# kamenbliznashki/chexpert

Measured on AMD Instinct MI355X. Metric: images/sec fwd+bwd DenseNet121 320x320 bf16 (per-GPU rate in config.images_per_sec_per_gpu), higher is better.
Workload: dtype bf16; 1 GPU; densenet121 bf16 1xMI355X 320x320 bs=256 per GPU, U-Ones labels (BASELINE configs[1]); 14 classes; random-init weights, synthetic uint8 X-rays; per_gpu_batch=256, global_batch=256, parallelism=dp1, rccl_ranks=1, capture_failed=0, launch=hipGraph replay

## Files before the change

chexpert_amd/csrc/conv3x3_ring.hip:

```cpp
#include <cstdlib>
#include <type_traits>
#include "common.h"

namespace {

constexpr int XP = 272;
constexpr int NT = 512;
constexpr int W_ROWS = 9 * 32;
constexpr int W_BYTES = W_ROWS * XP;
constexpr int RING_PX_MAX = (160 * 1024 - W_BYTES - 1024 - 256) / XP;

struct RingGeo {
  int B, H, W, P, R, Q;
  int Wt, ntx;
  int spi;
  int steps_per_wg;
  unsigned mP;
  unsigned mSpi;
  int ntx_shift;
};

__device__ __forceinline__ int wrapq(int v, int q) { return v >= q ? v - q : v; }
__device__ __forceinline__ int div_spi(const RingGeo& g, int v) { return g.spi == 1 ? v : (int)__umulhi((unsigned)v, g.mSpi); }

template <int CTRL>
__device__ __forceinline__ float dpp_add(float v) {
  return v + __int_as_float(__builtin_amdgcn_update_dpp(0, __float_as_int(v), CTRL, 0xF, 0xF, true));
}
__device__ __forceinline__ float half_sum(float v) {
  v = dpp_add<0xB1>(v);
  v = dpp_add<0x4E>(v);
  v = dpp_add<0x141>(v);
  v = dpp_add<0x140>(v);
  return v + __shfl_xor(v, 16);
}

#ifdef CX_RING_STAMPS
__device__ unsigned long long ring_stamps[1024 * 8];
__device__ unsigned long long ring_fwd_stamps[1024 * 8];
__device__ __forceinline__ unsigned long long rstamp() {
  unsigned long long t;
  __builtin_amdgcn_sched_barrier(0);
  asm volatile("s_memtime %0\n\ts_waitcnt lgkmcnt(0)" : "=s"(t)::"memory");
  __builtin_amdgcn_sched_barrier(0);
  return t;
}
#define RSTAMP(i) { const unsigned long long t_ = rstamp(); st_acc[i] += t_ - st_prev; st_prev = t_; }
#else
#define RSTAMP(i)
#endif
template <int NCH, int DEPTH>
__global__ __launch_bounds__(NT, 1) void conv3x3_ring_fwd_kernel(const bf16* __restrict__ x, int ldx, const float* __restrict__ sc,
                                                                const float* __restrict__ sh, const bf16* __restrict__ wpk,
                                                                bf16* __restrict__ y, int ldy, float* stat_sum, float* stat_sq,
                                                                int stat_replicas, int stat_rstride, int stat_det, const RingGeo g) {
  extern __shared__ __attribute__((aligned(16))) char smem[];
  float* coef = reinterpret_cast<float*>(smem);
  char* wl = smem + 1024 + 256;
  char* ring = wl + W_BYTES;
  const int tid = threadIdx.x, lane = tid & 63, wave = tid >> 6;
  const int lrow = lane & 31, lh = lane >> 5;
  const int P = g.P, R = g.R, Q = g.Q, W = g.W, H = g.H, Wt = g.Wt, ntx = g.ntx;

  for (int i = tid; i < W_ROWS * 16; i += NT) {
    const int row = i >> 4, c = i & 15;
    *reinterpret_cast<uint4*>(wl + row * XP + c * 16) = *reinterpret_cast<const uint4*>(wpk + (size_t)row * 128 + c * 8);
  }
  for (int i = tid; i < (Q + 2) * (XP / 16); i += NT) reinterpret_cast<uint4*>(ring)[i] = make_uint4(0, 0, 0, 0);
  __syncthreads();

  const int total_steps = g.B * g.spi;
  const int u0 = blockIdx.x * g.steps_per_wg;
  const int u1 = min(total_steps, u0 + g.steps_per_wg);
  const int chunks_per_row = P * 16;

  uint4 pre[DEPTH][NCH];
  bool pv[DEPTH][NCH];
  int base_row = 0;
  int crow[NCH], cpx[NCH];
  const int cc8 = tid & 15;
#pragma unroll
  for (int i = 0; i < NCH; ++i) {
    const int cid = tid + NT * i;
    crow[i] = cid / chunks_per_row;
    cpx[i] = (cid - crow[i] * chunks_per_row) >> 4;
  }
  float csc[8], csh[8];
#pragma unroll
  for (int j = 0; j < 8; ++j) { csc[j] = sc[cc8 * 8 + j]; csh[j] = sh[cc8 * 8 + j]; }
#pragma unroll
  for (int j = 0; j < 8; ++j) asm volatile("" ::"v"(csc[j]), "v"(csh[j]));
  uint32_t voff[NCH];
#pragma unroll
  for (int i = 0; i < NCH; ++i) voff[i] = ((uint32_t)(crow[i] * W + cpx[i]) * (uint32_t)ldx + (uint32_t)cc8 * 8u) * 2u;
  const char* __restrict__ xb = reinterpret_cast<const char*>(x);
  auto issue_rows = [&](uint4 (&pre)[NCH], bool (&pv)[NCH], int bv, int y0, int n) __attribute__((always_inline)) {
    const int b = bv >> g.ntx_shift, x0 = (bv - (b << g.ntx_shift)) * Wt - 1;
    const uint32_t sbase = (uint32_t)((b * H + y0) * W + x0) * (uint32_t)ldx * 2u;
    const uint32_t r_lo = (uint32_t)max(-y0, 0), r_n = (uint32_t)max(min(n, H - y0), 0) - r_lo;
    const uint32_t c_lo = (uint32_t)max(-x0, 0), c_n = (uint32_t)max(W - x0, 0) - c_lo;
#pragma unroll
    for (int i = 0; i < NCH; ++i) {
      pv[i] = ((uint32_t)crow[i] - r_lo) < r_n && ((uint32_t)cpx[i] - c_lo) < c_n;
      pre[i] = *reinterpret_cast<const uint4*>(xb + (size_t)(pv[i] ? sbase + voff[i] : 0u));
    }
  };
  auto write_rows = [&](uint4 (&pre)[NCH], bool (&pv)[NCH], int y0, int n) __attribute__((always_inline)) {
    int slot_y0 = (y0 - base_row) % (R + 2);
    if (slot_y0 < 0) slot_y0 += R + 2;
#pragma unroll
    for (int i = 0; i < NCH; ++i) {
      if (crow[i] < n) {
        int slot = slot_y0 + crow[i];
        if (slot >= R + 2) slot -= R + 2;
        U128 o;
        o.u = cx_affine_relu8(pre[i], csc, csh);
        { const unsigned keep = pv[i] ? 0xffffffffu : 0u; o.u.x &= keep; o.u.y &= keep; o.u.z &= keep; o.u.w &= keep; }
        const int pos = slot * P + cpx[i];
        *reinterpret_cast<uint4*>(ring + pos * XP + cc8 * 16) = o.u;
        if (pos < 2) *reinterpret_cast<uint4*>(ring + (Q + pos) * XP + cc8 * 16) = o.u;
      }
    }
  };
  int ulim = u1;
  auto issue_step = [&](uint4 (&pre)[NCH], bool (&pv)[NCH], int v) __attribute__((always_inline)) {
    const int bv = div_spi(g, v), sv = v - bv * g.spi;
    const bool ok = v < ulim && sv != 0;
    issue_rows(pre, pv, ok ? bv : 0, ok ? sv * R + 1 : 0, ok ? R : 0);
  };

  float s1[2][8], s2[2][8];
#pragma unroll
  for (int cc = 0; cc < 2; ++cc)
#pragma unroll
    for (int j = 0; j < 8; ++j) s1[cc][j] = s2[cc][j] = 0.f;
  const int nsub = (R * P + 31) / 32;
  const char* wbase = wl + lrow * XP + lh * 16;
#ifdef CX_RING_STAMPS
  unsigned long long st_acc[7] = {0, 0, 0, 0, 0, 0, 0}, st_prev = rstamp(), st_steps = 0;
#endif

  auto step = [&](int u, auto KI) __attribute__((always_inline)) {
    constexpr int k = decltype(KI)::value;
    uint4 (&cur)[NCH] = pre[k];
    bool (&cv)[NCH] = pv[k];
    const int bv = div_spi(g, u), yc = (u - bv * g.spi) * R;
    const int b = bv >> g.ntx_shift, x0 = (bv - (b << g.ntx_shift)) * Wt;
    RSTAMP(0)
    write_rows(cur, cv, yc + 1, R);
    RSTAMP(1)
    __syncthreads();
    RSTAMP(2)
    issue_step(cur, cv, u + DEPTH);
    RSTAMP(3)
    int slot0 = (yc - 1 - base_row) % (R + 2);
    if (slot0 < 0) slot0 += R + 2;
    const int ws = slot0 * P;

    for (int s = wave; s < nsub; s += NT / 64) {
      f32x16 acc;
#pragma unroll
      for (int r = 0; r < 16; ++r) acc[r] = 0.f;
      const int m = s * 32 + lrow;
      const int pix = min(m, R * P - 1);
      const char* ap0 = ring + wrapq(wrapq(ws + pix, Q), Q) * XP + lh * 16;
      const char* ap1 = ring + wrapq(wrapq(ws + pix + P, Q), Q) * XP + lh * 16;
      const char* ap2 = ring + wrapq(wrapq(ws + pix + 2 * P, Q), Q) * XP + lh * 16;
      constexpr int G = 3, NG = 72 / G;
      bf16x8 fa[3][G], fb[3][G];
      auto load_grp = [&](int gi, bf16x8 (&A)[G], bf16x8 (&B)[G]) __attribute__((always_inline)) {
#pragma unroll
        for (int j = 0; j < G; ++j) {
          const int f = gi * G + j, t = f >> 3, ks = f & 7;
          const int dy = t / 3, dx = t - dy * 3;
          A[j] = *reinterpret_cast<const bf16x8*>(wbase + t * 32 * XP + ks * 32);
          B[j] = *reinterpret_cast<const bf16x8*>((dy == 0 ? ap0 : dy == 1 ? ap1 : ap2) + dx * XP + ks * 32);
        }
      };
      load_grp(0, fa[0], fb[0]);
      load_grp(1, fa[1], fb[1]);
#pragma unroll
      for (int gi = 0; gi < NG; ++gi) {
        if (gi + 2 < NG) load_grp(gi + 2, fa[(gi + 2) % 3], fb[(gi + 2) % 3]);
        __builtin_amdgcn_sched_barrier(0);
#pragma unroll
        for (int j = 0; j < G; ++j)
          acc = __builtin_amdgcn_mfma_f32_32x32x16_bf16(fa[gi % 3][j], fb[gi % 3][j], acc, 0, 0, 0);
        __builtin_amdgcn_sched_barrier(0);
      }
#ifdef CX_RING_STAMPS
      asm volatile("" ::"v"(acc[0]));
#endif
      RSTAMP(4)
      const int oy = (int)__umulhi((unsigned)m, g.mP), ox = m - oy * P;
      const int yy = yc + oy;
      const bool valid = m < R * P && ox < Wt && x0 + ox < W && yy < H;
      bf16* yrow = y + ((size_t)(b * H + (valid ? yy : 0)) * W + (valid ? x0 + ox : 0)) * ldy;
#pragma unroll
      for (int cc = 0; cc < 2; ++cc) {
        U128 o;
        float t[8];
#pragma unroll
        for (int r4 = 0; r4 < 4; ++r4) {
          const auto sw = __builtin_amdgcn_permlane32_swap(__float_as_uint(acc[8 * cc + r4]), __float_as_uint(acc[8 * cc + 4 + r4]),
                                                           false, false);
          t[r4] = __uint_as_float(sw[0]);
          t[4 + r4] = __uint_as_float(sw[1]);
        }
        o.u = cx_pack8_stats(t, valid, true, s1[cc], s2[cc]);
        if (valid) *reinterpret_cast<uint4*>(yrow + 8 * (2 * cc + lh)) = o.u;
      }
      RSTAMP(5)
    }
    __syncthreads();
    RSTAMP(6)
#ifdef CX_RING_STAMPS
    ++st_steps;
#endif
  };

  const int rot = u1 - u0 > 1 ? (int)((blockIdx.x * 37u) % (unsigned)(u1 - u0)) : 0;
#pragma unroll 1
  for (int pass = 0; pass < 2; ++pass) {
  ulim = pass == 0 ? u1 : u0 + rot;
  for (int ui = pass == 0 ? u0 + rot : u0; ui < ulim;) {
    const int b = div_spi(g, ui), yc = (ui - b * g.spi) * R;
    const int ue = min(ulim, (b + 1) * g.spi);
    base_row = yc - 1;
    auto sync_rows = [&](int y0) __attribute__((always_inline)) {
      issue_rows(pre[0], pv[0], b, y0, 1);
      write_rows(pre[0], pv[0], y0, 1);
    };
    sync_rows(yc - 1);
    sync_rows(yc);
    issue_rows(pre[0], pv[0], b, yc + 1, R);
#pragma unroll
    for (int d = 1; d < DEPTH; ++d) issue_step(pre[d], pv[d], ui + d);
    for (int u = ui; u < ue; u += DEPTH) {
      step(u, std::integral_constant<int, 0>());
      if (DEPTH > 1) { if (u + 1 >= ue) break; step(u + 1, std::integral_constant<int, 1 % DEPTH>()); }
      if (DEPTH > 2) { if (u + 2 >= ue) break; step(u + 2, std::integral_constant<int, 2 % DEPTH>()); }
    }
    ui = ue;
  }
  }

#ifdef CX_RING_STAMPS
  if (tid == 0 && blockIdx.x < 1024) {
    for (int i = 0; i < 7; ++i) ring_fwd_stamps[blockIdx.x * 8 + i] = st_acc[i];
    ring_fwd_stamps[blockIdx.x * 8 + 7] = st_steps;
  }
#endif
  if (stat_sum) {
    float* scratch = reinterpret_cast<float*>(wl);
    wg_stat_begin<NT / 64>(scratch, 32, tid, NT);
    float t1 = 0.f, t2 = 0.f;
#pragma unroll
    for (int cc = 0; cc < 2; ++cc)
#pragma unroll
      for (int j = 0; j < 8; ++j) {
        const float a = half_sum(s1[cc][j]);
        const float c = half_sum(s2[cc][j]);
        if (lrow == 8 * cc + j) { t1 = a; t2 = c; }
      }
    if (lrow < 16) {
      const int n = 8 * (2 * (lrow >> 3) + lh) + (lrow & 7);
      wg_stat_put(scratch, 32, wave, n, t1, t2);
    }
    wg_stat_end<NT / 64>(scratch, 32, tid, NT, stat_sum, stat_sq, stat_det, (int)blockIdx.x, stat_replicas, stat_rstride, 0, 32);
  }
}

template <int NCH, int DEPTH>
int launch_ring(const CxConv& p, hipStream_t st, const RingGeo& g) {
  const size_t smem = 1024 + 256 + W_BYTES + (size_t)(g.Q + 2) * XP;
  static bool attr = false;
  if (!attr) {
    (void)hipFuncSetAttribute(reinterpret_cast<const void*>(&conv3x3_ring_fwd_kernel<NCH, DEPTH>), hipFuncAttributeMaxDynamicSharedMemorySize,
                              160 * 1024);
    attr = true;
  }
  const int total = g.B * g.spi;
  const int grid = (total + g.steps_per_wg - 1) / g.steps_per_wg;
  if (const int e = stat_rows_check(p, grid)) return e;
  CX_KTAG("conv3x3_ring_fwd_kernel<%d, %d>", NCH, DEPTH);
  hipLaunchKernelGGL((conv3x3_ring_fwd_kernel<NCH, DEPTH>), dim3(grid), dim3(NT), smem, st, (const bf16*)p.x, p.ldx, p.pa, p.pb,
                     (const bf16*)p.w, (bf16*)p.y, p.ldy, p.stat_sum, p.stat_sq, p.stat_replicas, p.stat_rstride, p.stat_det, g);
  return launch_status();
}


constexpr int GP = 80;
constexpr int DW_ROWS = 9 * 128;
constexpr int DW_BYTES = DW_ROWS * GP;
constexpr int EC_BYTES = 5 * 128 * 4 + 3 * 32 * 4;
constexpr int MAX_ITEMS = 2;

template <int NCH>
__global__ __launch_bounds__(NT, 1) void conv3x3_ring_dgrad_kernel(
    const bf16* __restrict__ gsl, int ldg, const bf16* __restrict__ g2, int ldg2, const float* __restrict__ ga,
    const float* __restrict__ gb, const float* __restrict__ gc, const bf16* __restrict__ wpk, const bf16* __restrict__ ex, int ldex,
    const float* __restrict__ e_sc, const float* __restrict__ e_sh, const float* __restrict__ e_mu, const float* __restrict__ e_r,
    const float* __restrict__ e_scale, bf16* __restrict__ y, int ldy, float* S1, float* S2, int stat_replicas, int stat_rstride,
    int stat_det, bf16* __restrict__ po, int ldpo, const RingGeo g) {
  extern __shared__ __attribute__((aligned(16))) char smem[];
  float* ecoef = reinterpret_cast<float*>(smem);
  char* wl = smem + EC_BYTES;
  char* ring = wl + DW_BYTES;
  const int tid = threadIdx.x, lane = tid & 63, wave = tid >> 6;
  const int lrow = lane & 31, lh = lane >> 5;
  const int h2 = wave & 1;
  const int P = g.P, R = g.R, Q = g.Q, W = g.W, H = g.H;

  for (int i = tid; i < DW_ROWS * 4; i += NT) {
    const int row = i >> 2, c = i & 3;
    *reinterpret_cast<uint4*>(wl + row * GP + c * 16) = *reinterpret_cast<const uint4*>(wpk + (size_t)row * 32 + c * 8);
  }
  for (int i = tid; i < (Q + 2) * (GP / 16); i += NT) reinterpret_cast<uint4*>(ring)[i] = make_uint4(0, 0, 0, 0);
  if (tid < 128) {
    ecoef[tid] = e_sc[tid]; ecoef[128 + tid] = e_sh[tid]; ecoef[256 + tid] = e_mu[tid]; ecoef[384 + tid] = e_r[tid];
    ecoef[512 + tid] = e_scale[tid];
  }
  if (tid < 32) { ecoef[640 + tid] = ga[tid]; ecoef[672 + tid] = gb[tid]; ecoef[704 + tid] = gc[tid]; }
  __syncthreads();

  const int total_steps = g.B * g.spi;
  const int u0 = blockIdx.x * g.steps_per_wg;
  const int u1 = min(total_steps, u0 + g.steps_per_wg);
  const int cpr = W * 4;

  uint4 pg[NCH], pg2[NCH];
  bool gv[NCH];
  int base_row = 0;
  int crow[NCH], cpx[NCH];
  const int cc4 = tid & 3;
#pragma unroll
  for (int i = 0; i < NCH; ++i) {
    const int cid = tid + NT * i;
    crow[i] = cid / cpr;
    cpx[i] = (cid - crow[i] * cpr) >> 2;
  }
  const float* kco = ecoef + 640 + cc4 * 8;

  uint32_t vog[NCH], vog2[NCH];
#pragma unroll
  for (int i = 0; i < NCH; ++i) {
    vog[i] = ((uint32_t)(crow[i] * W + cpx[i]) * (uint32_t)ldg + (uint32_t)cc4 * 8u) * 2u;
    vog2[i] = ((uint32_t)(crow[i] * W + cpx[i]) * (uint32_t)ldg2 + (uint32_t)cc4 * 8u) * 2u;
  }
  const char* __restrict__ gslb = reinterpret_cast<const char*>(gsl);
  const char* __restrict__ g2b = reinterpret_cast<const char*>(g2);
  auto issue_rows = [&](int b, int y0, int n) __attribute__((always_inline)) {
    const uint32_t row0 = (uint32_t)((b * H + y0) * W);
    const uint32_t sg = row0 * (uint32_t)ldg * 2u, sg2 = row0 * (uint32_t)ldg2 * 2u;
    const uint32_t r_lo = (uint32_t)max(-y0, 0), r_n = (uint32_t)max(min(n, H - y0), 0) - r_lo;
#pragma unroll
    for (int i = 0; i < NCH; ++i) {
      gv[i] = ((uint32_t)crow[i] - r_lo) < r_n;
      pg[i] = *reinterpret_cast<const uint4*>(gslb + (size_t)(gv[i] ? sg + vog[i] : 0u));
      pg2[i] = *reinterpret_cast<const uint4*>(g2b + (size_t)(gv[i] ? sg2 + vog2[i] : 0u));
    }
  };
  auto write_rows = [&](int b, int y0, int n) __attribute__((always_inline)) {
    int slot_y0 = (y0 - base_row) % (R + 2);
    if (slot_y0 < 0) slot_y0 += R + 2;
#pragma unroll
    for (int i = 0; i < NCH; ++i) {
      if (crow[i] < n) {
        int slot = slot_y0 + crow[i];
        if (slot >= R + 2) slot -= R + 2;
        U128 o;
        o.u = cx_affine2_8(pg[i], pg2[i], kco, kco + 32, kco + 64);
        if (po && gv[i]) *reinterpret_cast<uint4*>(po + ((size_t)(b * H + y0 + crow[i]) * W + cpx[i]) * ldpo + cc4 * 8) = o.u;
        { const unsigned keep = gv[i] ? 0xffffffffu : 0u; o.u.x &= keep; o.u.y &= keep; o.u.z &= keep; o.u.w &= keep; }
        const int pos = slot * P + cpx[i] + 1;
        *reinterpret_cast<uint4*>(ring + pos * GP + cc4 * 16) = o.u;
        if (pos < 2) *reinterpret_cast<uint4*>(ring + (Q + pos) * GP + cc4 * 16) = o.u;
      }
    }
  };

  float s1[2][2][8], s2[2][2][8];
#pragma unroll
  for (int j = 0; j < 2; ++j)
#pragma unroll
    for (int cc = 0; cc < 2; ++cc)
#pragma unroll
      for (int e = 0; e < 8; ++e) s1[j][cc][e] = s2[j][cc][e] = 0.f;
  const int nsub = (R * P + 31) / 32;
  const char* wbase = wl + (h2 * 64 + lrow) * GP + lh * 16;

#ifdef CX_RING_STAMPS
  unsigned long long st_acc[7] = {0, 0, 0, 0, 0, 0, 0}, st_prev = rstamp();
#endif
  for (int u = u0; u < u1; ++u) {
    const int b = div_spi(g, u), yc = (u - b * g.spi) * R;
    if (u == u0 || yc == 0) {
      base_row = yc - 1;
      issue_rows(b, yc - 1, 1);
      write_rows(b, yc - 1, 1);
      issue_rows(b, yc, 1);
      write_rows(b, yc, 1);
      issue_rows(b, yc + 1, R);
    }
    RSTAMP(0)
    write_rows(b, yc + 1, R);
    RSTAMP(1)
    __syncthreads();
    RSTAMP(2)
    const bool next_cont = (u + 1 < u1) && (div_spi(g, u + 1) == b);
    if (next_cont) issue_rows(b, yc + R + 1, R);
    RSTAMP(3)
    int slot0 = (yc - 1 - base_row) % (R + 2);
    if (slot0 < 0) slot0 += R + 2;
    const int ws = slot0 * P;

#pragma unroll 1
    for (int t = 0; t < MAX_ITEMS; ++t) {
      const int s = (wave >> 1) + 4 * t;
      if (s < nsub) {
        U128 xv[2][2];
        const int m = s * 32 + lrow;
        const int oy = (int)__umulhi((unsigned)m, g.mP), ox = m - oy * P;
        const int yy = yc + oy;
        const bool pok = m < R * P && ox < W && yy < H;
        const int poff = (b * H + min(yy, H - 1)) * W + min(ox, W - 1);
#pragma unroll
        for (int j = 0; j < 2; ++j)
#pragma unroll
          for (int cc = 0; cc < 2; ++cc)
            xv[j][cc].u = *reinterpret_cast<const uint4*>(ex + (size_t)poff * ldex + (2 * h2 + j) * 32 + 8 * (2 * cc + lh));
        f32x16 acc[2];
#pragma unroll
        for (int j = 0; j < 2; ++j)
#pragma unroll
          for (int r = 0; r < 16; ++r) acc[j][r] = 0.f;
        const int pix = min(s * 32 + lrow, R * P - 1);
        const char* ap0 = ring + wrapq(wrapq(ws + pix, Q), Q) * GP + lh * 16;
        const char* ap1 = ring + wrapq(wrapq(ws + pix + P, Q), Q) * GP + lh * 16;
        const char* ap2 = ring + wrapq(wrapq(ws + pix + 2 * P, Q), Q) * GP + lh * 16;
        bf16x8 fb[2][2], fa[2][2][2];
        auto load_tap = [&](int t, bf16x8 (&B)[2], bf16x8 (&A)[2][2]) __attribute__((always_inline)) {
          const int dy = t / 3, dx = t - dy * 3;
          const char* ap = (dy == 0 ? ap0 : dy == 1 ? ap1 : ap2) + dx * GP;
          const char* wp = wbase + t * 128 * GP;
#pragma unroll
          for (int ks = 0; ks < 2; ++ks) {
            B[ks] = *reinterpret_cast<const bf16x8*>(ap + ks * 32);
#pragma unroll
            for (int j = 0; j < 2; ++j) A[ks][j] = *reinterpret_cast<const bf16x8*>(wp + (j * 32) * GP + ks * 32);
          }
        };
        load_tap(0, fb[0], fa[0]);
#pragma unroll
        for (int t = 0; t < 9; ++t) {
          if (t + 1 < 9) load_tap(t + 1, fb[(t + 1) & 1], fa[(t + 1) & 1]);
          __builtin_amdgcn_sched_barrier(0);
#pragma unroll
          for (int ks = 0; ks < 2; ++ks)
#pragma unroll
            for (int j = 0; j < 2; ++j)
              acc[j] = __builtin_amdgcn_mfma_f32_32x32x16_bf16(fa[t & 1][ks][j], fb[t & 1][ks], acc[j], 0, 0, 0);
          __builtin_amdgcn_sched_barrier(0);
        }
#ifdef CX_RING_STAMPS
        asm volatile("" ::"v"(acc[0][0]), "v"(acc[1][0]));
#endif
        RSTAMP(4)
        bf16* yrow = y + (size_t)poff * ldy;
#pragma unroll
        for (int j = 0; j < 2; ++j)
#pragma unroll
          for (int cc = 0; cc < 2; ++cc) {
            const int n = (2 * h2 + j) * 32 + 8 * (2 * cc + lh);
            float v[8];
#pragma unroll
            for (int r4 = 0; r4 < 4; ++r4) {
              const auto sw = __builtin_amdgcn_permlane32_swap(__float_as_uint(acc[j][8 * cc + r4]),
                                                               __float_as_uint(acc[j][8 * cc + 4 + r4]), false, false);
              v[r4] = __uint_as_float(sw[0]);
              v[4 + r4] = __uint_as_float(sw[1]);
            }
            float xf[8], dz[8];
            {
              asm volatile("" ::: "memory");
              const float4 a0 = *reinterpret_cast<const float4*>(ecoef + n), a1 = *reinterpret_cast<const float4*>(ecoef + n + 4);
              const float4 b0 = *reinterpret_cast<const float4*>(ecoef + 128 + n), b1 = *reinterpret_cast<const float4*>(ecoef + 128 + n + 4);
              const float esc[8] = {a0.x, a0.y, a0.z, a0.w, a1.x, a1.y, a1.z, a1.w};
              const float esh[8] = {b0.x, b0.y, b0.z, b0.w, b1.x, b1.y, b1.z, b1.w};
              const uint32_t xw[4] = {xv[j][cc].u.x, xv[j][cc].u.y, xv[j][cc].u.z, xv[j][cc].u.w};
#pragma unroll
              for (int e = 0; e < 8; ++e) {
                xf[e] = (e & 1) ? cx_bf_hi(xw[e >> 1]) : cx_bf_lo(xw[e >> 1]);
                dz[e] = (pok && fmaf(xf[e], esc[e], esh[e]) > 0.f) ? v[e] : 0.f;
                s1[j][cc][e] += dz[e];
              }
            }
#pragma unroll
            for (int e = 0; e < 8; ++e) s2[j][cc][e] = fmaf(dz[e], xf[e], s2[j][cc][e]);
            U128 o;
            {
              asm volatile("" ::: "memory");
              const float4 e0 = *reinterpret_cast<const float4*>(ecoef + 512 + n), e1 = *reinterpret_cast<const float4*>(ecoef + 512 + n + 4);
              const float esl[8] = {e0.x, e0.y, e0.z, e0.w, e1.x, e1.y, e1.z, e1.w};
              o.u = make_uint4(cx_packbf(esl[0] * dz[0], esl[1] * dz[1]), cx_packbf(esl[2] * dz[2], esl[3] * dz[3]),
                               cx_packbf(esl[4] * dz[4], esl[5] * dz[5]), cx_packbf(esl[6] * dz[6], esl[7] * dz[7]));
            }
            if (pok) *reinterpret_cast<uint4*>(yrow + n) = o.u;
          }
        RSTAMP(5)
      }
    }
    __syncthreads();
    RSTAMP(6)
  }
#ifdef CX_RING_STAMPS
  if (tid == 0 && blockIdx.x < 1024) {
    for (int i = 0; i < 7; ++i) ring_stamps[blockIdx.x * 8 + i] = st_acc[i];
    ring_stamps[blockIdx.x * 8 + 7] = (unsigned long long)(u1 - u0);
  }
#endif

  {
    float* scratch = reinterpret_cast<float*>(wl);
    wg_stat_begin<NT / 64>(scratch, 128, tid, NT);
#pragma unroll
    for (int j = 0; j < 2; ++j) {
      float t1 = 0.f, t2 = 0.f;
#pragma unroll
      for (int cc = 0; cc < 2; ++cc)
#pragma unroll
        for (int e = 0; e < 8; ++e) {
          const float a = half_sum(s1[j][cc][e]);
          const float c = half_sum(s2[j][cc][e]);
          if (lrow == 8 * cc + e) { t1 = a; t2 = c; }
        }
      if (lrow < 16) {
        const int n = (2 * h2 + j) * 32 + 8 * (2 * (lrow >> 3) + lh) + (lrow & 7);
        wg_stat_put(scratch, 128, wave, n, t1, ecoef[384 + n] * (t2 - ecoef[256 + n] * t1));
      }
    }
    wg_stat_end<NT / 64>(scratch, 128, tid, NT, S1, S2, stat_det, (int)blockIdx.x, stat_replicas, stat_rstride, 0, 128);
  }
}

template <int NCH>
int launch_ring_dgrad(const CxConv& p, hipStream_t st, const RingGeo& g) {
  const size_t smem = EC_BYTES + DW_BYTES + (size_t)(g.Q + 2) * GP;
  static bool attr = false;
  if (!attr) {
    (void)hipFuncSetAttribute(reinterpret_cast<const void*>(&conv3x3_ring_dgrad_kernel<NCH>), hipFuncAttributeMaxDynamicSharedMemorySize,
                              160 * 1024);
    attr = true;
  }
  const int total = g.B * g.spi;
  const int grid = (total + g.steps_per_wg - 1) / g.steps_per_wg;
  if (const int e = stat_rows_check(p, grid)) return e;
  CX_KTAG("conv3x3_ring_dgrad_kernel<%d>", NCH);
  hipLaunchKernelGGL((conv3x3_ring_dgrad_kernel<NCH>), dim3(grid), dim3(NT), smem, st, (const bf16*)p.x, p.ldx, (const bf16*)p.x2,
                     p.ldx2, p.pa, p.pb, p.pc, (const bf16*)p.w, (const bf16*)p.ex, p.ldex, p.e_sc, p.e_sh, p.e_mu, p.e_r, p.e_scale,
                     (bf16*)p.y, p.ldy, p.stat_sum, p.stat_sq, p.stat_replicas, p.stat_rstride, p.stat_det, (bf16*)p.pro_out, p.ldpo, g);
  cx_tl_pro_out = p.pro_out ? 1 : 0;
  return launch_status();
}


constexpr int WNT = 768;
constexpr int WXP = 320;
constexpr int WGP = 64;
constexpr int WCOEF = 352 * 4;

__device__ __forceinline__ bf16x8 tr2(const char* a0, const char* a1) {
  typedef __attribute__((address_space(3))) s16x4 lds_s16x4;
  return cx_join_tr(__builtin_amdgcn_ds_read_tr16_b64_v4i16((lds_s16x4*)(a0)), __builtin_amdgcn_ds_read_tr16_b64_v4i16((lds_s16x4*)(a1)));
}

template <int NX, int NG>
__global__ __launch_bounds__(WNT, 1) void conv3x3_ring_wgrad_kernel(
    const bf16* __restrict__ gsl, int ldg, const bf16* __restrict__ g2, int ldg2, const float* __restrict__ ga,
    const float* __restrict__ gb, const float* __restrict__ gc, int g_affine2, const bf16* __restrict__ x, int ldx,
    const float* __restrict__ pa, const float* __restrict__ pb, float* __restrict__ dw, const RingGeo g,
    float* __restrict__ slab) {
  extern __shared__ __attribute__((aligned(16))) char smem[];
  const int P = g.P, R = g.R, Q = g.Q, W = g.W, H = g.H;
  const int nk = (R * P + 15) / 16;
  float* coef = reinterpret_cast<float*>(smem);
  char* ring = smem + WCOEF;
  char* gst = ring + (size_t)(Q + 2) * WXP;
  float* red = reinterpret_cast<float*>(ring);
  const int tid = threadIdx.x, lane = tid & 63, wave = tid >> 6;
  const int cs = wave & 3, dy = wave >> 2;

  for (int i = tid; i < ((Q + 2) * WXP + nk * 16 * WGP) / 16; i += WNT) reinterpret_cast<uint4*>(ring)[i] = make_uint4(0, 0, 0, 0);
  if (tid < 128) { coef[tid] = pa[tid]; coef[128 + tid] = pb[tid]; }
  if (tid < 32) {
    coef[256 + tid] = g_affine2 ? ga[tid] : 1.f;
// ... 250 lines not shown
  return need <= 1 ? launch_ring_dgrad<1>(p, st, g) : launch_ring_dgrad<2>(p, st, g);
}

int cx_try_ring_wgrad(const CxWgrad& p, hipStream_t st, bool* handled) {
  *handled = false;
  if (p.mode != CX_MODE_CONV || p.kh != 3 || p.kw != 3 || p.stride != 1 || p.pad != 1) return 0;
  if (p.K != 128 || p.N != 32 || p.x_prologue != CX_PRO_AFFINE_RELU) return 0;
  if (p.g_prologue != CX_PRO_NONE && p.g_prologue != CX_PRO_AFFINE2) return 0;
  if (p.W < 56 || (long long)p.H * p.W < 3136) return 0;
  {
    const unsigned long long ldm = (unsigned long long)(p.ldx > p.ldg ? p.ldx : p.ldg) > (unsigned long long)p.ldg2 ? (unsigned long long)(p.ldx > p.ldg ? p.ldx : p.ldg) : (unsigned long long)p.ldg2;
    if ((unsigned long long)p.B * p.H * p.W * ldm * 2ull >= (1ull << 32)) return 0;
  }
  RingGeo g;
  g.B = p.B; g.H = p.H; g.W = p.W; g.P = p.W + 2;
  int rmax = 0;
  for (int r = 1; r <= p.H; ++r) {
    const int nk = (r * g.P + 15) / 16;
    const size_t bytes = WCOEF + (size_t)((r + 2) * g.P + 2) * WXP + (size_t)nk * 16 * WGP;
    if (nk > 16 || bytes > 160 * 1024 || r * p.W * 16 > 5 * WNT || r * p.W * 4 > 2 * WNT) break;
    rmax = r;
  }
  if (rmax < 1) return 0;
  g.spi = (p.H + rmax - 1) / rmax;
  g.R = (p.H + g.spi - 1) / g.spi;
  g.spi = (p.H + g.R - 1) / g.R;
  g.Q = (g.R + 2) * g.P;
  g.mP = 0xffffffffu / (unsigned)g.P + 1u;
  g.mSpi = 0xffffffffu / (unsigned)g.spi + 1u;
  g.ntx_shift = 0;
  if ((unsigned long long)p.B * 2ull * g.spi * g.spi >= (1ull << 32)) return 0;
  const int nk = (g.R * g.P + 15) / 16;
  size_t smem = WCOEF + (size_t)(g.Q + 2) * WXP + (size_t)nk * 16 * WGP;
  if (smem < WCOEF + 32 * 288 * 4) smem = WCOEF + 32 * 288 * 4;
  const int total = g.B * g.spi;
  int spw = (total + 255) / 256;
  if (g.B >= 256) spw = ((g.B + 255) / 256) * g.spi;
  if (spw < 1) spw = 1;
  g.steps_per_wg = spw;
  const int nx = (g.R * p.W * 16 + WNT - 1) / WNT, ng = (g.R * p.W * 4 + WNT - 1) / WNT;
  *handled = true;
  if (nx <= 2 && ng <= 1) return launch_ring_wgrad<2, 1>(p, st, g, smem);
  if (nx <= 3) return launch_ring_wgrad<3, 2>(p, st, g, smem);
  return launch_ring_wgrad<5, 2>(p, st, g, smem);
}

#ifdef CX_RING_STAMPS
extern "C" int dbg_ring_stamps(unsigned long long* host, int n_words) {
  return (int)hipMemcpyFromSymbol(host, HIP_SYMBOL(ring_stamps), (size_t)n_words * 8, 0, hipMemcpyDeviceToHost);
}
extern "C" int dbg_ring_fwd_stamps(unsigned long long* host, int n_words) {
  return (int)hipMemcpyFromSymbol(host, HIP_SYMBOL(ring_fwd_stamps), (size_t)n_words * 8, 0, hipMemcpyDeviceToHost);
}
#endif
```

scratch/stamps_ring.py:

```python
import ctypes, os, shutil, sys, numpy as np, torch
sys.path.insert(0, '.')
from chexpert_amd import _lib
shutil.copy("scratch/libstamp_ring.so", _lib.LIB_PATH)
from chexpert_amd import ops
dev = torch.device('cuda:0'); bf = torch.bfloat16; B = 256
names = ["restart", "wait+stage", "barrier1", "issue", "items:multiply", "items:epilogue", "barrier2"]
for hw, ctot in ((80, 256), (40, 512), (20, 1024)):
    z1 = (torch.randn(B, hw, hw, 128, device=dev) * 0.5).to(bf)
    buf = (torch.randn(B, hw, hw, ctot, device=dev) * 0.5).to(bf)
    gbuf = (torch.randn(B, hw, hw, ctot, device=dev) * 0.5).to(bf)
    dz = torch.empty(B, hw, hw, 128, device=dev, dtype=bf)
    w = (torch.randn(9 * 32 * 128, device=dev) * 0.05).to(bf)
    one, zero = torch.ones(128, device=dev), torch.zeros(128, device=dev)
    cap = 4096
    st = torch.zeros(2, cap * 128, device=dev)
    ys, gs = buf[..., 64:96], gbuf[..., 64:96]
    d = lambda: ops.conv_gemm(gs, w, dz, N=128, kh=3, kw=3, pad=1, prologue=ops.PRO_AFFINE2, x2=ys, pa=one[:32], pb=zero[:32], pc=zero[:32],
                              epilogue=ops.EPI_MASK, ex=z1, e_sc=one, e_sh=zero, e_mu=zero, e_r=one, e_scale=one, stat_sum=st[0], stat_sq=st[1],
                              stat_det=True, stat_replicas=cap, stat_rstride=128)
    one128 = torch.ones(128, device=dev); zero128 = torch.zeros(128, device=dev)
    f = lambda: ops.conv_gemm(z1, w, ys, N=32, kh=3, kw=3, pad=1, prologue=ops.PRO_AFFINE_RELU, pa=one128, pb=zero128, stat_sum=st[0], stat_sq=st[1],
                              stat_det=True, stat_replicas=cap, stat_rstride=32)
    for _ in range(3): f()
    torch.cuda.synchronize()
    e0, e1 = torch.cuda.Event(enable_timing=True), torch.cuda.Event(enable_timing=True)
    e0.record(); f(); e1.record(); torch.cuda.synchronize()
    kname = _lib.lib().cx_last_kernel().decode()
    host = (ctypes.c_ulonglong * (1024 * 8))()
    ctypes.CDLL(_lib.LIB_PATH).dbg_ring_fwd_stamps(host, 1024 * 8)
    a = np.frombuffer(host, dtype=np.uint64).reshape(1024, 8).astype(np.float64)[:256]
    a = a[a[:, 7] > 0]
    med = np.median(a[:, :7] / a[:, 7:8], 0)
    fn = ["between steps", "wait+stage", "barrier1", "issue", "sub-tiles:multiply", "sub-tiles:epilogue", "barrier2"]
    print("%dx%d FORWARD (%s, %.1f us): steps/wg %.0f, core clocks per step %.0f: " % (hw, hw, kname, e0.elapsed_time(e1) * 1e3, np.median(a[:, 7]), med.sum()) +
          ", ".join("%s %.0f" % (nm, v) for nm, v in zip(fn, med)), flush=True)
    for _ in range(3): d()
    torch.cuda.synchronize()
    e0, e1 = torch.cuda.Event(enable_timing=True), torch.cuda.Event(enable_timing=True)
    e0.record(); d(); e1.record(); torch.cuda.synchronize()
    host = (ctypes.c_ulonglong * (1024 * 8))()
    ctypes.CDLL(_lib.LIB_PATH).dbg_ring_stamps(host, 1024 * 8)
    a = np.frombuffer(host, dtype=np.uint64).reshape(1024, 8).astype(np.float64)
    a = a[:256]
    a = a[a[:, 7] > 0]
    per = a[:, :7] / a[:, 7:8]
    med = np.median(per, 0)
    print("%dx%d (%s, %.1f us): steps/wg %.0f, core clocks per step %.0f: " % (hw, hw, _lib.lib().cx_last_kernel().decode(), e0.elapsed_time(e1) * 1e3, np.median(a[:, 7]), med.sum()) +
          ", ".join("%s %.0f" % (nm, v) for nm, v in zip(names, med)), flush=True)
```

Measured before the change: 9363 images/sec.

## Overlap ring conv prologue loads with weight staging and batch halo-row restarts

The forward and backward 3x3 ring conv kernels now load weights into registers first, issue the first halo and body row loads before writing weights to LDS, and drop the initial barrier and full ring zero-fill (the backward kernel only zeroes pad columns). Restart staging issues both halo rows in one batch when they fit, instead of a serial issue-then-write per row. The per-column stat reduction becomes a transpose-style butterfly using DPP and ds_swizzle that reduces 16 values at once, replacing 16 separate half-sums. Optional prologue timing stamps are added behind a debug macro. The risks are correctness, since the initial barrier and ring zeroing are gone, and extra register pressure from the held weight and halo registers.

```diff
diff --git a/chexpert_amd/csrc/conv3x3_ring.hip b/chexpert_amd/csrc/conv3x3_ring.hip
--- a/chexpert_amd/csrc/conv3x3_ring.hip
+++ b/chexpert_amd/csrc/conv3x3_ring.hip
@@ -24,15 +24,20 @@
 __device__ __forceinline__ int div_spi(const RingGeo& g, int v) { return g.spi == 1 ? v : (int)__umulhi((unsigned)v, g.mSpi); }
 
 template <int CTRL>
-__device__ __forceinline__ float dpp_add(float v) {
-  return v + __int_as_float(__builtin_amdgcn_update_dpp(0, __float_as_int(v), CTRL, 0xF, 0xF, true));
-}
-__device__ __forceinline__ float half_sum(float v) {
-  v = dpp_add<0xB1>(v);
-  v = dpp_add<0x4E>(v);
-  v = dpp_add<0x141>(v);
-  v = dpp_add<0x140>(v);
-  return v + __shfl_xor(v, 16);
+__device__ __forceinline__ float dpp_get(float v) { return __int_as_float(__builtin_amdgcn_update_dpp(0, __float_as_int(v), CTRL, 0xF, 0xF, true)); }
+template <int XOR>
+__device__ __forceinline__ float swz_xor(float v) { return __int_as_float(__builtin_amdgcn_ds_swizzle(__float_as_int(v), (XOR << 10) | 0x1F)); }
+__device__ __forceinline__ float half_sum16(const float (&v)[16], int lane) {
+  const bool b0 = lane & 1, b1 = lane & 2, b2 = lane & 4, b3 = lane & 8;
+  float a[8], b[4], c[2];
+#pragma unroll
+  for (int k = 0; k < 8; ++k) a[k] = (b0 ? v[2 * k + 1] : v[2 * k]) + dpp_get<0xB1>(b0 ? v[2 * k] : v[2 * k + 1]);
+#pragma unroll
+  for (int k = 0; k < 4; ++k) b[k] = (b1 ? a[2 * k + 1] : a[2 * k]) + dpp_get<0x4E>(b1 ? a[2 * k] : a[2 * k + 1]);
+#pragma unroll
+  for (int k = 0; k < 2; ++k) c[k] = (b2 ? b[2 * k + 1] : b[2 * k]) + swz_xor<4>(b2 ? b[2 * k] : b[2 * k + 1]);
+  const float d = (b3 ? c[1] : c[0]) + swz_xor<8>(b3 ? c[0] : c[1]);
+  return d + swz_xor<16>(d);
 }
 
 #ifdef CX_RING_STAMPS
@@ -46,8 +51,23 @@
   return t;
 }
 #define RSTAMP(i) { const unsigned long long t_ = rstamp(); st_acc[i] += t_ - st_prev; st_prev = t_; }
+__device__ unsigned long long ring_pro_stamps[1024 * 8];
+__device__ unsigned long long ring_fwd_pro_stamps[1024 * 8];
+#define PSTAMP_BEGIN unsigned long long ps_acc[3] = {0, 0, 0}; const unsigned long long ps_rt0 = __builtin_amdgcn_s_memrealtime(), ps_t0 = rstamp(); \
+  unsigned long long ps_prev = ps_t0; bool ps_first = true;
+#define PSTAMP(i) { const unsigned long long t_ = rstamp(); ps_acc[i] = t_ - ps_prev; ps_prev = t_; }
+#define PSTAMP_FIRST_MFMA if (ps_first) { PSTAMP(1) ps_first = false; }
+#define PSTAMP_MARK ps_prev = rstamp();
+#define PSTAMP_END(arr) { PSTAMP(2) const unsigned long long rt_ = __builtin_amdgcn_s_memrealtime(); \
+  if (threadIdx.x == 0 && blockIdx.x < 1024) { for (int i = 0; i < 3; ++i) arr[blockIdx.x * 8 + i] = ps_acc[i]; \
+    arr[blockIdx.x * 8 + 3] = ps_prev - ps_t0; arr[blockIdx.x * 8 + 4] = rt_ - ps_rt0; } }
 #else
 #define RSTAMP(i)
+#define PSTAMP_BEGIN
+#define PSTAMP(i)
+#define PSTAMP_FIRST_MFMA
+#define PSTAMP_MARK
+#define PSTAMP_END(arr)
 #endif
 template <int NCH, int DEPTH>
 __global__ __launch_bounds__(NT, 1) void conv3x3_ring_fwd_kernel(const bf16* __restrict__ x, int ldx, const float* __restrict__ sc,
@@ -61,14 +81,17 @@
   const int tid = threadIdx.x, lane = tid & 63, wave = tid >> 6;
   const int lrow = lane & 31, lh = lane >> 5;
   const int P = g.P, R = g.R, Q = g.Q, W = g.W, H = g.H, Wt = g.Wt, ntx = g.ntx;
-
-  for (int i = tid; i < W_ROWS * 16; i += NT) {
-    const int row = i >> 4, c = i & 15;
-    *reinterpret_cast<uint4*>(wl + row * XP + c * 16) = *reinterpret_cast<const uint4*>(wpk + (size_t)row * 128 + c * 8);
-  }
-  for (int i = tid; i < (Q + 2) * (XP / 16); i += NT) reinterpret_cast<uint4*>(ring)[i] = make_uint4(0, 0, 0, 0);
-  __syncthreads();
-
+  PSTAMP_BEGIN
+
+  static_assert((W_ROWS * 16) % NT == 0, "whole weight chunks per thread");
+  constexpr int WCH = W_ROWS * 16 / NT;
+  uint4 wv[WCH];
+#pragma unroll
+  for (int j = 0; j < WCH; ++j) {
+    const int i = tid + NT * j;
+    wv[j] = *reinterpret_cast<const uint4*>(wpk + (size_t)(i >> 4) * 128 + (i & 15) * 8);
+  }
+  __builtin_amdgcn_sched_barrier(0);
   const int total_steps = g.B * g.spi;
   const int u0 = blockIdx.x * g.steps_per_wg;
   const int u1 = min(total_steps, u0 + g.steps_per_wg);
@@ -76,6 +99,9 @@
 
   uint4 pre[DEPTH][NCH];
   bool pv[DEPTH][NCH];
+  constexpr int HN = NCH < 3 ? NCH : 3;
+  uint4 hal[HN];
+  bool hv[HN];
   int base_row = 0;
   int crow[NCH], cpx[NCH];
   const int cc8 = tid & 15;
@@ -88,28 +114,28 @@
   float csc[8], csh[8];
 #pragma unroll
   for (int j = 0; j < 8; ++j) { csc[j] = sc[cc8 * 8 + j]; csh[j] = sh[cc8 * 8 + j]; }
-#pragma unroll
-  for (int j = 0; j < 8; ++j) asm volatile("" ::"v"(csc[j]), "v"(csh[j]));
   uint32_t voff[NCH];
 #pragma unroll
   for (int i = 0; i < NCH; ++i) voff[i] = ((uint32_t)(crow[i] * W + cpx[i]) * (uint32_t)ldx + (uint32_t)cc8 * 8u) * 2u;
   const char* __restrict__ xb = reinterpret_cast<const char*>(x);
-  auto issue_rows = [&](uint4 (&pre)[NCH], bool (&pv)[NCH], int bv, int y0, int n) __attribute__((always_inline)) {
+  auto issue_rows = [&](auto& pre, auto& pv, int bv, int y0, int n, int ns) __attribute__((always_inline)) {
+    constexpr int NS = (int)(sizeof(pv) / sizeof(pv[0]));
     const int b = bv >> g.ntx_shift, x0 = (bv - (b << g.ntx_shift)) * Wt - 1;
     const uint32_t sbase = (uint32_t)((b * H + y0) * W + x0) * (uint32_t)ldx * 2u;
     const uint32_t r_lo = (uint32_t)max(-y0, 0), r_n = (uint32_t)max(min(n, H - y0), 0) - r_lo;
     const uint32_t c_lo = (uint32_t)max(-x0, 0), c_n = (uint32_t)max(W - x0, 0) - c_lo;
 #pragma unroll
-    for (int i = 0; i < NCH; ++i) {
+    for (int i = 0; i < NS; ++i) {
       pv[i] = ((uint32_t)crow[i] - r_lo) < r_n && ((uint32_t)cpx[i] - c_lo) < c_n;
-      pre[i] = *reinterpret_cast<const uint4*>(xb + (size_t)(pv[i] ? sbase + voff[i] : 0u));
-    }
-  };
-  auto write_rows = [&](uint4 (&pre)[NCH], bool (&pv)[NCH], int y0, int n) __attribute__((always_inline)) {
+      if (i < ns) pre[i] = *reinterpret_cast<const uint4*>(xb + (size_t)(pv[i] ? sbase + voff[i] : 0u));
+    }
+  };
+  auto write_rows = [&](auto& pre, auto& pv, int y0, int n, int P) __attribute__((always_inline)) {
+    constexpr int NS = (int)(sizeof(pv) / sizeof(pv[0]));
     int slot_y0 = (y0 - base_row) % (R + 2);
     if (slot_y0 < 0) slot_y0 += R + 2;
 #pragma unroll
-    for (int i = 0; i < NCH; ++i) {
+    for (int i = 0; i < NS; ++i) {
       if (crow[i] < n) {
         int slot = slot_y0 + crow[i];
         if (slot >= R + 2) slot -= R + 2;
@@ -126,8 +152,56 @@
   auto issue_step = [&](uint4 (&pre)[NCH], bool (&pv)[NCH], int v) __attribute__((always_inline)) {
     const int bv = div_spi(g, v), sv = v - bv * g.spi;
     const bool ok = v < ulim && sv != 0;
-    issue_rows(pre, pv, ok ? bv : 0, ok ? sv * R + 1 : 0, ok ? R : 0);
-  };
+    issue_rows(pre, pv, ok ? bv : 0, ok ? sv * R + 1 : 0, ok ? R : 0, NCH);
+  };
+  const bool halo2 = 2 * chunks_per_row <= HN * NT;
+  const int halo_ns = (2 * chunks_per_row + NT - 1) / NT;
+  auto issue_refill = [&](int ui, int b, int yc) __attribute__((always_inline)) {
+    issue_rows(pre[0], pv[0], b, yc + 1, R, NCH);
+#pragma unroll
+    for (int d = 1; d < DEPTH; ++d) issue_step(pre[d], pv[d], ui + d);
+  };
+  auto restart_issue = [&](int ui) __attribute__((always_inline)) {
+    const int b = div_spi(g, ui), yc = (ui - b * g.spi) * R;
+    if (halo2) {
+      issue_rows(hal, hv, b, yc - 1, 2, halo_ns);
+      issue_refill(ui, b, yc);
+    } else if constexpr (DEPTH == 1) {
+      issue_rows(pre[0], pv[0], b, yc - 1, 2, NCH);
+    } else {
+      issue_rows(pre[1], pv[1], b, yc - 1, 1, NCH);
+      issue_rows(pre[0], pv[0], b, yc, 1, NCH);
+    }
+  };
+  auto restart_stage = [&](int ui) __attribute__((always_inline)) {
+    const int b = div_spi(g, ui), yc = (ui - b * g.spi) * R;
+    base_row = yc - 1;
+    int n1 = 1, n2 = 2, Pq = P;
+    asm volatile("" : "+s"(n1), "+s"(n2), "+s"(Pq));
+    if (halo2) {
+      write_rows(hal, hv, yc - 1, n2, Pq);
+    } else {
+      if constexpr (DEPTH == 1) {
+        write_rows(pre[0], pv[0], yc - 1, n2, Pq);
+      } else {
+        write_rows(pre[1], pv[1], yc - 1, n1, Pq);
+        write_rows(pre[0], pv[0], yc, n1, Pq);
+      }
+      issue_refill(ui, b, yc);
+    }
+  };
+
+  const int rot = u1 - u0 > 1 ? (int)((blockIdx.x * 37u) % (unsigned)(u1 - u0)) : 0;
+  restart_issue(u0 + rot);
+  __builtin_amdgcn_sched_barrier(0);
+#pragma unroll
+  for (int j = 0; j < WCH; ++j) {
+    const int i = tid + NT * j;
+    *reinterpret_cast<uint4*>(wl + (i >> 4) * XP + (i & 15) * 16) = wv[j];
+  }
+#pragma unroll
+  for (int j = 0; j < 8; ++j) asm volatile("" ::"v"(csc[j]), "v"(csh[j]));
+  PSTAMP(0)
 
   float s1[2][8], s2[2][8];
 #pragma unroll
@@ -147,12 +221,13 @@
     const int bv = div_spi(g, u), yc = (u - bv * g.spi) * R;
     const int b = bv >> g.ntx_shift, x0 = (bv - (b << g.ntx_shift)) * Wt;
     RSTAMP(0)
-    write_rows(cur, cv, yc + 1, R);
+    write_rows(cur, cv, yc + 1, R, P);
     RSTAMP(1)
     __syncthreads();
     RSTAMP(2)
     issue_step(cur, cv, u + DEPTH);
     RSTAMP(3)
+    PSTAMP_FIRST_MFMA
     int slot0 = (yc - 1 - base_row) % (R + 2);
     if (slot0 < 0) slot0 += R + 2;
     const int ws = slot0 * P;
@@ -219,23 +294,16 @@
 #endif
   };
 
-  const int rot = u1 - u0 > 1 ? (int)((blockIdx.x * 37u) % (unsigned)(u1 - u0)) : 0;
+  bool first = true;
 #pragma unroll 1
   for (int pass = 0; pass < 2; ++pass) {
   ulim = pass == 0 ? u1 : u0 + rot;
   for (int ui = pass == 0 ? u0 + rot : u0; ui < ulim;) {
-    const int b = div_spi(g, ui), yc = (ui - b * g.spi) * R;
+    const int b = div_spi(g, ui);
     const int ue = min(ulim, (b + 1) * g.spi);
-    base_row = yc - 1;
-    auto sync_rows = [&](int y0) __attribute__((always_inline)) {
-      issue_rows(pre[0], pv[0], b, y0, 1);
-      write_rows(pre[0], pv[0], y0, 1);
-    };
-    sync_rows(yc - 1);
-    sync_rows(yc);
-    issue_rows(pre[0], pv[0], b, yc + 1, R);
-#pragma unroll
-    for (int d = 1; d < DEPTH; ++d) issue_step(pre[d], pv[d], ui + d);
+    if (!first) restart_issue(ui);
+    first = false;
+    restart_stage(ui);
     for (int u = ui; u < ue; u += DEPTH) {
       step(u, std::integral_constant<int, 0>());
       if (DEPTH > 1) { if (u + 1 >= ue) break; step(u + 1, std::integral_constant<int, 1 % DEPTH>()); }
@@ -244,6 +312,7 @@
     ui = ue;
   }
   }
+  PSTAMP_MARK
 
 #ifdef CX_RING_STAMPS
   if (tid == 0 && blockIdx.x < 1024) {
@@ -253,22 +322,20 @@
 #endif
   if (stat_sum) {
     float* scratch = reinterpret_cast<float*>(wl);
-    wg_stat_begin<NT / 64>(scratch, 32, tid, NT);
-    float t1 = 0.f, t2 = 0.f;
+    float f1[16], f2[16];
 #pragma unroll
     for (int cc = 0; cc < 2; ++cc)
 #pragma unroll
-      for (int j = 0; j < 8; ++j) {
-        const float a = half_sum(s1[cc][j]);
-        const float c = half_sum(s2[cc][j]);
-        if (lrow == 8 * cc + j) { t1 = a; t2 = c; }
-      }
+      for (int j = 0; j < 8; ++j) { f1[8 * cc + j] = s1[cc][j]; f2[8 * cc + j] = s2[cc][j]; }
+    const float t1 = half_sum16(f1, lane), t2 = half_sum16(f2, lane);
     if (lrow < 16) {
       const int n = 8 * (2 * (lrow >> 3) + lh) + (lrow & 7);
-      wg_stat_put(scratch, 32, wave, n, t1, t2);
+      scratch[(wave * 2) * 32 + n] = t1;
+      scratch[(wave * 2 + 1) * 32 + n] = t2;
     }
     wg_stat_end<NT / 64>(scratch, 32, tid, NT, stat_sum, stat_sq, stat_det, (int)blockIdx.x, stat_replicas, stat_rstride, 0, 32);
   }
+  PSTAMP_END(ring_fwd_pro_stamps)
 }
 
 template <int NCH, int DEPTH>
@@ -311,19 +378,17 @@
   const int lrow = lane & 31, lh = lane >> 5;
   const int h2 = wave & 1;
   const int P = g.P, R = g.R, Q = g.Q, W = g.W, H = g.H;
-
-  for (int i = tid; i < DW_ROWS * 4; i += NT) {
-    const int row = i >> 2, c = i & 3;
-    *reinterpret_cast<uint4*>(wl + row * GP + c * 16) = *reinterpret_cast<const uint4*>(wpk + (size_t)row * 32 + c * 8);
-  }
-  for (int i = tid; i < (Q + 2) * (GP / 16); i += NT) reinterpret_cast<uint4*>(ring)[i] = make_uint4(0, 0, 0, 0);
-  if (tid < 128) {
-    ecoef[tid] = e_sc[tid]; ecoef[128 + tid] = e_sh[tid]; ecoef[256 + tid] = e_mu[tid]; ecoef[384 + tid] = e_r[tid];
-    ecoef[512 + tid] = e_scale[tid];
-  }
-  if (tid < 32) { ecoef[640 + tid] = ga[tid]; ecoef[672 + tid] = gb[tid]; ecoef[704 + tid] = gc[tid]; }
-  __syncthreads();
-
+  PSTAMP_BEGIN
+
+  static_assert((DW_ROWS * 4) % NT == 0, "whole weight chunks per thread");
+  constexpr int WCH = DW_ROWS * 4 / NT;
+  uint4 wv[WCH];
+#pragma unroll
+  for (int j = 0; j < WCH; ++j) {
+    const int i = tid + NT * j;
+    wv[j] = *reinterpret_cast<const uint4*>(wpk + (size_t)(i >> 2) * 32 + (i & 3) * 8);
+  }
+  __builtin_amdgcn_sched_barrier(0);
   const int total_steps = g.B * g.spi;
   const int u0 = blockIdx.x * g.steps_per_wg;
   const int u1 = min(total_steps, u0 + g.steps_per_wg);
@@ -331,6 +396,8 @@
 
   uint4 pg[NCH], pg2[NCH];
   bool gv[NCH];
+  uint4 hg[NCH], hg2[NCH];
+  bool hgv[NCH];
   int base_row = 0;
   int crow[NCH], cpx[NCH];
   const int cc4 = tid & 3;
@@ -340,7 +407,11 @@
     crow[i] = cid / cpr;
     cpx[i] = (cid - crow[i] * cpr) >> 2;
   }
-  const float* kco = ecoef + 640 + cc4 * 8;
+  float* kco = ecoef + 640 + cc4 * 8;
+  float ev[5], kv[3][8];
+  if (tid < 128) { ev[0] = e_sc[tid]; ev[1] = e_sh[tid]; ev[2] = e_mu[tid]; ev[3] = e_r[tid]; ev[4] = e_scale[tid]; }
+#pragma unroll
+  for (int j = 0; j < 8; ++j) { kv[0][j] = ga[cc4 * 8 + j]; kv[1][j] = gb[cc4 * 8 + j]; kv[2][j] = gc[cc4 * 8 + j]; }
 
   uint32_t vog[NCH], vog2[NCH];
 #pragma unroll
@@ -350,7 +421,7 @@
   }
   const char* __restrict__ gslb = reinterpret_cast<const char*>(gsl);
   const char* __restrict__ g2b = reinterpret_cast<const char*>(g2);
-  auto issue_rows = [&](int b, int y0, int n) __attribute__((always_inline)) {
+  auto issue_rows = [&](uint4 (&pg)[NCH], uint4 (&pg2)[NCH], bool (&gv)[NCH], int b, int y0, int n) __attribute__((always_inline)) {
     const uint32_t row0 = (uint32_t)((b * H + y0) * W);
     const uint32_t sg = row0 * (uint32_t)ldg * 2u, sg2 = row0 * (uint32_t)ldg2 * 2u;
     const uint32_t r_lo = (uint32_t)max(-y0, 0), r_n = (uint32_t)max(min(n, H - y0), 0) - r_lo;
@@ -361,7 +432,7 @@
       pg2[i] = *reinterpret_cast<const uint4*>(g2b + (size_t)(gv[i] ? sg2 + vog2[i] : 0u));
     }
   };
-  auto write_rows = [&](int b, int y0, int n) __attribute__((always_inline)) {
+  auto write_rows = [&](uint4 (&pg)[NCH], uint4 (&pg2)[NCH], bool (&gv)[NCH], int b, int y0, int n, int P) __attribute__((always_inline)) {
     int slot_y0 = (y0 - base_row) % (R + 2);
     if (slot_y0 < 0) slot_y0 += R + 2;
 #pragma unroll
@@ -379,6 +450,50 @@
       }
     }
   };
+  const bool halo2 = 2 * cpr <= NCH * NT;
+  auto restart_issue = [&](int b, int yc) __attribute__((always_inline)) {
+    if (halo2) {
+      issue_rows(hg, hg2, hgv, b, yc - 1, 2);
+      issue_rows(pg, pg2, gv, b, yc + 1, R);
+    } else {
+      issue_rows(hg, hg2, hgv, b, yc - 1, 1);
+      issue_rows(pg, pg2, gv, b, yc, 1);
+    }
+  };
+  auto restart_stage = [&](int b, int yc) __attribute__((always_inline)) {
+    base_row = yc - 1;
+    int n1 = 1, n2 = 2, Pq = P;
+    asm volatile("" : "+s"(n1), "+s"(n2), "+s"(Pq));
+    if (halo2) {
+      write_rows(hg, hg2, hgv, b, yc - 1, n2, Pq);
+    } else {
+      write_rows(hg, hg2, hgv, b, yc - 1, n1, Pq);
+      write_rows(pg, pg2, gv, b, yc, n1, Pq);
+      issue_rows(pg, pg2, gv, b, yc + 1, R);
+    }
+  };
+
+  {
+    const int b0 = div_spi(g, u0);
+    restart_issue(b0, (u0 - b0 * g.spi) * R);
+  }
+  __builtin_amdgcn_sched_barrier(0);
+#pragma unroll
+  for (int j = 0; j < WCH; ++j) {
+    const int i = tid + NT * j;
+    *reinterpret_cast<uint4*>(wl + (i >> 2) * GP + (i & 3) * 16) = wv[j];
+  }
+#pragma unroll
+  for (int j = 0; j < 8; ++j) { kco[j] = kv[0][j]; kco[32 + j] = kv[1][j]; kco[64 + j] = kv[2][j]; }
+  if (tid < 128) {
+    ecoef[tid] = ev[0]; ecoef[128 + tid] = ev[1]; ecoef[256 + tid] = ev[2]; ecoef[384 + tid] = ev[3]; ecoef[512 + tid] = ev[4];
+  }
+  for (int i = tid; i < (2 * (R + 2) + 1) * 4; i += NT) {
+    const int k = i >> 2;
+    const int pos = k == 2 * (R + 2) ? Q : (k >> 1) * P + (k & 1) * (P - 1);
+    *reinterpret_cast<uint4*>(ring + pos * GP + (i & 3) * 16) = make_uint4(0, 0, 0, 0);
+  }
+  PSTAMP(0)
 
   float s1[2][2][8], s2[2][2][8];
 #pragma unroll
@@ -396,21 +511,18 @@
   for (int u = u0; u < u1; ++u) {
     const int b = div_spi(g, u), yc = (u - b * g.spi) * R;
     if (u == u0 || yc == 0) {
-      base_row = yc - 1;
-      issue_rows(b, yc - 1, 1);
-      write_rows(b, yc - 1, 1);
-      issue_rows(b, yc, 1);
-      write_rows(b, yc, 1);
-      issue_rows(b, yc + 1, R);
+      if (u != u0) restart_issue(b, yc);
+      restart_stage(b, yc);
     }
     RSTAMP(0)
-    write_rows(b, yc + 1, R);
+    write_rows(pg, pg2, gv, b, yc + 1, R, P);
     RSTAMP(1)
     __syncthreads();
     RSTAMP(2)
     const bool next_cont = (u + 1 < u1) && (div_spi(g, u + 1) == b);
-    if (next_cont) issue_rows(b, yc + R + 1, R);
+    if (next_cont) issue_rows(pg, pg2, gv, b, yc + R + 1, R);
     RSTAMP(3)
+    PSTAMP_FIRST_MFMA
     int slot0 = (yc - 1 - base_row) % (R + 2);
     if (slot0 < 0) slot0 += R + 2;
     const int ws = slot0 * P;
@@ -514,6 +626,7 @@
     __syncthreads();
     RSTAMP(6)
   }
+  PSTAMP_MARK
 #ifdef CX_RING_STAMPS
   if (tid == 0 && blockIdx.x < 1024) {
     for (int i = 0; i < 7; ++i) ring_stamps[blockIdx.x * 8 + i] = st_acc[i];
@@ -523,25 +636,25 @@
 
   {
     float* scratch = reinterpret_cast<float*>(wl);
-    wg_stat_begin<NT / 64>(scratch, 128, tid, NT);
 #pragma unroll
     for (int j = 0; j < 2; ++j) {
-      float t1 = 0.f, t2 = 0.f;
+      float f1[16], f2[16];
 #pragma unroll
       for (int cc = 0; cc < 2; ++cc)
 #pragma unroll
-        for (int e = 0; e < 8; ++e) {
-          const float a = half_sum(s1[j][cc][e]);
-          const float c = half_sum(s2[j][cc][e]);
-          if (lrow == 8 * cc + e) { t1 = a; t2 = c; }
-        }
+        for (int e = 0; e < 8; ++e) { f1[8 * cc + e] = s1[j][cc][e]; f2[8 * cc + e] = s2[j][cc][e]; }
+      const float t1 = half_sum16(f1, lane), t2 = half_sum16(f2, lane);
       if (lrow < 16) {
         const int n = (2 * h2 + j) * 32 + 8 * (2 * (lrow >> 3) + lh) + (lrow & 7);
-        wg_stat_put(scratch, 128, wave, n, t1, ecoef[384 + n] * (t2 - ecoef[256 + n] * t1));
+        scratch[(wave * 2) * 128 + n] = t1;
+        scratch[(wave * 2 + 1) * 128 + n] = ecoef[384 + n] * (t2 - ecoef[256 + n] * t1);
+        scratch[(wave * 2) * 128 + (n ^ 64)] = 0.f;
+        scratch[(wave * 2 + 1) * 128 + (n ^ 64)] = 0.f;
       }
     }
     wg_stat_end<NT / 64>(scratch, 128, tid, NT, S1, S2, stat_det, (int)blockIdx.x, stat_replicas, stat_rstride, 0, 128);
   }
+  PSTAMP_END(ring_pro_stamps)
 }
 
 template <int NCH>
@@ -898,4 +1011,8 @@
 extern "C" int dbg_ring_fwd_stamps(unsigned long long* host, int n_words) {
   return (int)hipMemcpyFromSymbol(host, HIP_SYMBOL(ring_fwd_stamps), (size_t)n_words * 8, 0, hipMemcpyDeviceToHost);
 }
+extern "C" int dbg_ring_pro_stamps(unsigned long long* host, int n_words, int fwd) {
+  return fwd ? (int)hipMemcpyFromSymbol(host, HIP_SYMBOL(ring_fwd_pro_stamps), (size_t)n_words * 8, 0, hipMemcpyDeviceToHost)
+             : (int)hipMemcpyFromSymbol(host, HIP_SYMBOL(ring_pro_stamps), (size_t)n_words * 8, 0, hipMemcpyDeviceToHost);
+}
 #endif
diff --git a/scratch/stamps_ring.py b/scratch/stamps_ring.py
--- a/scratch/stamps_ring.py
+++ b/scratch/stamps_ring.py
@@ -1,11 +1,20 @@
 import ctypes, os, shutil, sys, numpy as np, torch
 sys.path.insert(0, '.')
 from chexpert_amd import _lib
-shutil.copy("scratch/libstamp_ring.so", _lib.LIB_PATH)
+shutil.copy(sys.argv[1] if len(sys.argv) > 1 else "scratch/libstamp_ring.so", _lib.LIB_PATH)
 from chexpert_amd import ops
 dev = torch.device('cuda:0'); bf = torch.bfloat16; B = 256
 names = ["restart", "wait+stage", "barrier1", "issue", "items:multiply", "items:epilogue", "barrier2"]
-for hw, ctot in ((80, 256), (40, 512), (20, 1024)):
+def outside(fwd):
+    host = (ctypes.c_ulonglong * (1024 * 8))()
+    ctypes.CDLL(_lib.LIB_PATH).dbg_ring_pro_stamps(host, 1024 * 8, fwd)
+    a = np.frombuffer(host, dtype=np.uint64).reshape(1024, 8).astype(np.float64)[:256]
+    a = a[a[:, 4] > 0]
+    m = np.median(a, 0)
+    mhz = np.median(a[:, 3] / a[:, 4]) * 100.0
+    return "   outside the loop, clocks per launch at %.0f MHz: setup %.0f (%.2f us), setup -> first MFMA %.0f (%.2f us), last step -> end %.0f (%.2f us), kernel %.0f (%.2f us)" % (
+        mhz, m[0], m[0] / mhz, m[1], m[1] / mhz, m[2], m[2] / mhz, m[3], m[3] / mhz)
+for hw, ctot in ((80, 256), (40, 512), (20, 1024), (10, 1024)):
     z1 = (torch.randn(B, hw, hw, 128, device=dev) * 0.5).to(bf)
     buf = (torch.randn(B, hw, hw, ctot, device=dev) * 0.5).to(bf)
     gbuf = (torch.randn(B, hw, hw, ctot, device=dev) * 0.5).to(bf)
@@ -34,6 +43,7 @@
     fn = ["between steps", "wait+stage", "barrier1", "issue", "sub-tiles:multiply", "sub-tiles:epilogue", "barrier2"]
     print("%dx%d FORWARD (%s, %.1f us): steps/wg %.0f, core clocks per step %.0f: " % (hw, hw, kname, e0.elapsed_time(e1) * 1e3, np.median(a[:, 7]), med.sum()) +
           ", ".join("%s %.0f" % (nm, v) for nm, v in zip(fn, med)), flush=True)
+    print(outside(1), flush=True)
     for _ in range(3): d()
     torch.cuda.synchronize()
     e0, e1 = torch.cuda.Event(enable_timing=True), torch.cuda.Event(enable_timing=True)
@@ -47,3 +57,4 @@
     med = np.median(per, 0)
     print("%dx%d (%s, %.1f us): steps/wg %.0f, core clocks per step %.0f: " % (hw, hw, _lib.lib().cx_last_kernel().decode(), e0.elapsed_time(e1) * 1e3, np.median(a[:, 7]), med.sum()) +
           ", ".join("%s %.0f" % (nm, v) for nm, v in zip(names, med)), flush=True)
+    print(outside(0), flush=True)
```

Result: faster. 9546 images/sec, median of 6 (+2.0%).
